# truemeat001/Simple-Raytracing-Render

Measured on AMD Instinct MI355X. Metric: Msamples/s (rays x bounces) + HBM GB/s vs roofline, Cornell+teapot 1024spp, higher is better.
Workload: dtype f32

## Files before the change

simple-raytracing-render_amd/csrc/kernels.h:

```cpp
#pragma once
#include <hip/hip_runtime.h>

#include <cstdint>

#include "device_scene.h"

namespace srr {

struct SceneView {
  const DObj* objs;
  int n_world;
  int has_media;
  const DXform* xforms;
  const DSphere* spheres;
  const DRect* rects;
  const DStandaloneTri* stris;
  const DMesh* meshes;
  const float4* nodes;
  const float4* node4;
  int node4_lds;
  int node4_total;
  const float4* node4q;
  int node4_lds_q;
  int use_q;
// ... 72 lines not shown
  UDiv31 div_spp, div_nx;
  uint64_t base_seed;
  int64_t n_paths;
  int max_depth;
  unsigned long long* cursor;
  unsigned long long* counters;
  float* sample;
  float* raw;
  uint8_t* rays;
  int keep_spp, keep_s0;
  float4* rec;
  int lanes;
  int* err;
  int stack_cap;
  int2* gstack;
  int gstack_cap;
  unsigned long long* wave_times;
  int deep_tries;
  float* slow_rays;
  unsigned* slow_count;
  int walk_q;
};
#ifndef SRR_KSTACK
#define SRR_KSTACK 8
#endif
constexpr int kPathsLdsStack = SRR_KSTACK;
constexpr int kPathsGlobalStack = 56;

constexpr int kPathsWorldLdsBytes = 8192;
#ifndef SRR_LDS_NODES
#define SRR_LDS_NODES 96
#endif
constexpr int kPathsLdsNodes = SRR_LDS_NODES;
void dump_trace_timing();
int paths_lanes_per_device(const SceneView& S, int device);
int paths_block_lanes(const SceneView& S);
int launch_paths(const SceneView& S, const PathWork& W, int all_families, hipStream_t st);
struct KatTables {
  const DCamera* cams;
  const DRect* rects;
  const DSphere* spheres;
  const DStandaloneTri* stris;
  const DLight* lights;
  int n_lights;
  const DObj* objs;
  const DXform* xforms;
  const DMedium* media;
  const DMat* mats;
  const DTex* texs;
  const uint8_t* images;
  const float* perlin_ranvec;
  const int32_t* perlin_perm;
  const int32_t* base;
};
int launch_kat(int kind, int n, int w, float* d_rec, const float* d_aux, const DStandaloneTri* d_tris,
               const KatTables& kt);
enum LibmId : int {
  kLibmRsin, kLibmRcos, kLibmRexp, kLibmRlog, kLibmRpow, kLibmRacos, kLibmRasin, kLibmRatan2, kLibmRdiv,
  kLibmSincosf, kLibmAtanf, kLibmSin64, kLibmCos64, kLibmSincos64, kLibmAcos64, kLibmAtan2_64, kLibmLog64,
  kLibmOcmlLog, kLibmOcmlSin, kLibmOcmlCos, kLibmOcmlPow5
};
struct LibmFn {
  LibmId id;
  const char* name;
  int f64, n_in, n_out;
};
// ... 61 lines not shown
```

simple-raytracing-render_amd/csrc/kernels.hip:

```cpp
#include <hip/hip_runtime.h>

#include <cfloat>
#include <algorithm>
#include <cstdint>
#include <cstdlib>
#include <cstring>

#include "device_scene.h"
#include "devmath.h"
#include "kernels.h"
#include "../../include/srr/merl.h"

namespace srr {
namespace dev {

SRR_D V3 sphere_center(const DSphere& s, float tm, bool moving) {
  V3 c0 = v3(s.c0[0], s.c0[1], s.c0[2]);
  if (!moving) return c0;
  V3 c1 = v3(s.c1[0], s.c1[1], s.c1[2]);
  return c0 + ((tm - s.t0) / (s.t1 - s.t0)) * (c1 - c0);
}

SRR_D bool sphere_hit(const DSphere& s, bool moving, const Ray& r, float tmin, float tmax, float& t) {
  V3 oc = r.o - sphere_center(s, r.tm, moving);
// ... 2524 lines not shown
      emitted = hit_emitted(S, mat, rdir, v3(hp.x, hp.y, hp.z), v3(hn.x, hn.y, hn.z), hp.w, hn.w);
    }
    finish_path(P, p, emitted, depth, spec, max_depth);
    return false;
  }
  float4 hp = ntl(&P.hit_p[p]), hn = ntl(&P.hit_n[p]);
  V3 hpt = v3(hp.x, hp.y, hp.z), nrm = v3(hn.x, hn.y, hn.z);
  const DMat M = S.mats[mat];
  Rng rng{ntl(&P.lcg[p]), ntl(&P.pcg[p])};
  V3 ndir;
  float ntime;
  float4 rec;
  bool sp;
  scatter<F>(S, M, rdir, ro.w, hpt, nrm, hp.w, hn.w, rng, rec, sp, ndir, ntime);
  nts(&P.rec_a[(size_t)p * max_depth + depth], rec);
  if (sp) spec |= (1ull << depth);
  nts(&P.ray_o[p], make_float4(hpt.x, hpt.y, hpt.z, ntime));
  nts(&P.ray_d[p], make_float4(ndir.x, ndir.y, ndir.z, 0.f));
  nts(&P.lcg[p], rng.lcg);
  nts(&P.pcg[p], rng.pcg);
  nts(&P.depth[p], depth + 1);
  nts(&P.spec[p], spec);
  return true;
}

SRR_D float4 rec_load(const float4* p) { return *p; }

constexpr int kPathsBlock = 256;
constexpr unsigned long long kPoolChunk = 64;

#ifndef SRR_DIAG_VARIANTS
#define SRR_DIAG_VARIANTS 0
#endif
constexpr int kRingWords = 11;

constexpr int kPathsLdsNodesBig =
    (160 * 1024 - 8192 - 8 * kPathsLdsStack * 1024 - 1024 - 4 * kRingWords * 1024) / 128;
constexpr int kPathsLdsNodesSmall = 8;

SRR_D void path_camera_ray(const SceneView& S, const PathWork& W, uint32_t idx, Ray& r, Rng& rng) {
  const uint32_t lp = udiv31(idx, W.div_spp), s = idx - lp * (uint32_t)W.spp_w;
  if ((int)lp >= W.npix || (int)s >= W.spp_w) atomicOr(W.err, 1);
  const int pix = W.pixels ? W.pixels[lp] : lp;
  V3 o, d;
  float tm;
  double sx, sy;
  sobol2_point((uint32_t)(W.s_base + (int)s), sx, sy);
  camera_ray(S, pix, W.s_base + s, sx, sy, W.nx, W.ny, W.base_seed, o, d, tm, rng, &W.div_nx);
  r = Ray{o, d, tm};
}

template <int BS>
SRR_D void ring_put(lds_ptr<float> e, const Ray& r, const Rng& rng) {
  e[0] = r.o.x;
  e[BS] = r.o.y;
  e[2 * BS] = r.o.z;
  e[3 * BS] = r.d.x;
  e[4 * BS] = r.d.y;
  e[5 * BS] = r.d.z;
  e[6 * BS] = r.tm;
  e[7 * BS] = __uint_as_float((uint32_t)rng.lcg);
  e[8 * BS] = __uint_as_float((uint32_t)(rng.lcg >> 32));
  e[9 * BS] = __uint_as_float((uint32_t)rng.pcg);
  e[10 * BS] = __uint_as_float((uint32_t)(rng.pcg >> 32));
}

template <int BS>
SRR_D void ring_get(lds_ptr<const float> e, Ray& r, Rng& rng) {
  r = Ray{v3(e[0], e[BS], e[2 * BS]), v3(e[3 * BS], e[4 * BS], e[5 * BS]), e[6 * BS]};
  rng.lcg = (uint64_t)__float_as_uint(e[7 * BS]) | ((uint64_t)__float_as_uint(e[8 * BS]) << 32);
  rng.pcg = (uint64_t)__float_as_uint(e[9 * BS]) | ((uint64_t)__float_as_uint(e[10 * BS]) << 32);
}

struct PathsArgs {
  SceneView S;
  PathWork W;
};
#if defined(__HIP_DEVICE_COMPILE__)
template <class T>
using kptr = const __attribute__((address_space(4))) T*;
SRR_D kptr<PathsArgs> paths_args() {
  kptr<PathsArgs> p = (kptr<PathsArgs>)__builtin_amdgcn_kernarg_segment_ptr();
  asm volatile("" : "+s"(p));
  return p;
}
#else
SRR_D const PathsArgs* paths_args() { return nullptr; }
#endif

template <bool MEDIA, bool ALLFAM, int MINB, bool TIMED = false, bool WL = true, bool QUAD = false, bool CQ = false,
          int BS = kPathsBlock, bool SP = false>
#ifdef SRR_NUM_VGPR
#define SRR_PATHS_VGPR_ATTR __attribute__((amdgpu_num_vgpr(SRR_NUM_VGPR)))
#else
#define SRR_PATHS_VGPR_ATTR
#endif
__global__ void __launch_bounds__(BS, MINB) SRR_PATHS_VGPR_ATTR k_paths(PathsArgs A) {
  static_assert(BS == kPathsBlock || BS == 1024, "block size");
  (void)A;
  uint64_t tp[8] = {0, 0, 0, 0, 0, 0, 0, 0};
  uint64_t tf[20] = {0, 0, 0, 0, 0, 0, 0, 0, 0, 0, 0, 0, 0, 0, 0, 0, 0, 0, 0, 0};
  uint64_t it = 0;
  constexpr int TR = TR_BVH4_PRUNE | (WL ? TR_WL : 0) | (QUAD ? TR_QUAD : 0) | (CQ ? TR_Q : 0) | (BS == 1024 ? TR_BIG : 0) |
                     ((SP && !QUAD && !CQ) ? TR_SUSP : 0);
  __shared__ uint4 s_world[WL ? kWorldLdsBytes / 16 : 1];
  const auto view = [&]() {
    SceneView S = paths_args()->S;
    if constexpr (WL) {
      const char* b = (const char*)s_world;
      S.objs = (const DObj*)(b + S.world_off[0]);
      S.xforms = (const DXform*)(b + S.world_off[1]);
      S.spheres = (const DSphere*)(b + S.world_off[2]);
      S.rects = (const DRect*)(b + S.world_off[3]);
      S.stris = (const DStandaloneTri*)(b + S.world_off[4]);
      S.meshes = (const DMesh*)(b + S.world_off[5]);
      S.media = (const DMedium*)(b + S.world_off[6]);
      S.mats = (const DMat*)(b + S.world_off[7]);
      S.texs = (const DTex*)(b + S.world_off[8]);
      S.lights = (const DLight*)(b + S.world_off[9]);
    }
    return S;
  };
  const auto work = []() { return PathWork(paths_args()->W); };
  __shared__ int s_node[kStack * BS];
  __shared__ float s_t[kStack * BS];
  constexpr bool RING = !QUAD;
  constexpr int kNodesLds = BS == 1024 ? kPathsLdsNodesBig : ((WL && RING) ? kPathsLdsNodesSmall : kPathsLdsNodes);
  __shared__ float4 s_n4[kNodesLds * 8];
  __shared__ float s_ring[RING ? kRingWords * BS : 1];
  const lds_ptr<float> ringw = to_lds(s_ring + (RING ? (threadIdx.x & ~63u) : 0));
  uint32_t ring_base = 0;
  const uint32_t n_paths = (uint32_t)paths_args()->W.n_paths;
  const uint64_t t_start = paths_args()->W.wave_times ? __builtin_amdgcn_s_memrealtime() : 0;
  {
    const SceneView S0 = paths_args()->S;
    if constexpr (WL)
      for (int i = threadIdx.x; i < S0.world_words; i += blockDim.x) s_world[i] = S0.world_blob[i];
    const int n_lds_nodes = CQ ? min(S0.node4_total, 2 * kNodesLds) : min(S0.node4_total, kNodesLds);
    if (CQ)
      for (int i = threadIdx.x; i < n_lds_nodes * 4; i += blockDim.x) s_n4[i] = S0.node4q[i];
    else
      for (int i = threadIdx.x; i < n_lds_nodes * 8; i += blockDim.x) s_n4[i] = S0.node4[i];
  }
  __syncthreads();
  const int slot = blockIdx.x * blockDim.x + threadIdx.x;
  const auto rec_at = [&](const PathWork& W, int k) -> float4* {
    int s = slot;
    asm volatile("" : "+v"(s));
    return W.rec + ((size_t)k * W.lanes + s);
  };
  int g = -1;
  uint32_t pool = 0, pool_end = 0;
  uint32_t nxt_lane0 = 0;
  bool nxt_armed = false;
  uint32_t nxt_base = 0;
  bool nxt_ready = false;
  Ray r{};
  Rng rng{};
  int depth = 0;
  int walking = 0;
  uint32_t nrays = 0;
  uint32_t n_events = 0;
  constexpr uint32_t kCapped = 1, kSuspended = 1u << 12;
  uint32_t n_iter = 0, max_rounds = 0;
  for (;;) {
    ++n_iter;
    uint64_t tq = TIMED ? __builtin_amdgcn_s_memtime() : 0;
    const bool need = g < 0;
    const uint64_t nm = __ballot(need);
    if (nm && pool < n_paths) {
      const SceneView S = view();
      const PathWork W = work();
      const uint32_t cnt = __popcll(nm);
      const uint32_t rank = __popcll(nm & ((1ull << lane_id()) - 1));
      const uint32_t avail = pool_end - pool;
      uint32_t idx = 0;
      if (RING) {
        if (need && rank < avail) {
          const uint32_t i0 = pool + rank;
          if (i0 < n_paths) {
            g = (int)i0;
            ring_get<BS>(ringw + (i0 - ring_base), r, rng);
            depth = 0;
          }
        }
        if (avail >= cnt) {
          pool += cnt;
        } else {
          uint32_t nb;
          if (nxt_armed) {
            nb = nxt_ready ? nxt_base : __builtin_amdgcn_readfirstlane(nxt_lane0);
            nxt_armed = false;
            nxt_ready = false;
          } else {
            uint32_t b = 0;
            if (lane_id() == 0) b = (uint32_t)atomicAdd(W.cursor, (unsigned long long)kPoolChunk);
            nb = __builtin_amdgcn_readfirstlane(b);
          }
          const uint32_t gi = nb + (uint32_t)lane_id();
          if (gi < n_paths) {
// ... 22 lines not shown
        uint32_t nb;
        if (nxt_armed) {
          nb = nxt_ready ? nxt_base : __builtin_amdgcn_readfirstlane(nxt_lane0);
          nxt_armed = false;
          nxt_ready = false;
        } else {
          uint32_t b = 0;
          if (lane_id() == 0) b = (uint32_t)atomicAdd(W.cursor, (unsigned long long)kPoolChunk);
          nb = __builtin_amdgcn_readfirstlane(b);
        }
        idx = rank < avail ? pool + rank : nb + (rank - avail);
        pool = nb + (cnt - avail);
        pool_end = nb + (uint32_t)kPoolChunk;
      }
      if (!RING && need && idx < n_paths) {
        g = (int)idx;
        path_camera_ray(S, W, idx, r, rng);
        depth = 0;
      }
    }
    if (!nxt_armed && pool_end < n_paths) {
      if (lane_id() == 0) nxt_lane0 = (uint32_t)atomicAdd(paths_args()->W.cursor, (unsigned long long)kPoolChunk);
      nxt_armed = true;
    }
    if (__ballot(g >= 0) == 0) break;
    if (TIMED) tf[9] += __popcll(__ballot(g >= 0));
    if (TIMED) {
      __builtin_amdgcn_s_waitcnt(0);
      const uint64_t t = __builtin_amdgcn_s_memtime();
      tp[0] += t - tq;
      tq = t;
      ++it;
    }
    bool done = false;
    V3 C = v3(0.f);
    bool diff = false, pend = false;
    int natt = 0;
    uint64_t fam_dt[3] = {0, 0, 0};
    DiffSetup ds{};
    V3 d_atten = v3(0.f), d_n = v3(0.f), d_dir = v3(0.f);
    float d_pdf = 0;
    int d_tries = 0;
    bool d_dead = false;
    WorldHit w{-1, -1, 0};
    if (g >= 0) {
      const SceneView S = view();
      const PathWork W = work();
      TraceCtx cx{nullptr, to_lds(s_node + threadIdx.x), to_lds(s_t + threadIdx.x)};
      cx.lds_nodes = (const __attribute__((address_space(3))) f32x4*)to_lds(s_n4);
      cx.lds_count = CQ ? min(S.node4_total, 2 * kNodesLds) : min(S.node4_total, kNodesLds);
      cx.st_cap = min(W.stack_cap, kStack);
      cx.ovf = W.counters + 11;
      cx.gst = W.gstack;
      cx.gst_cap = W.gstack ? W.gstack_cap : 0;
      cx.gst_stride = W.lanes;
      cx.slot = slot;
      if constexpr ((TR & TR_SUSP) != 0) {
        cx.walk_thr = vreg((int)((__popcll(__ballot(true)) * (uint32_t)paths_args()->W.walk_q) >> 6));
        cx.resume = walking;
        cx.susp = vreg(0);
      }
#ifdef SRR_SLOW_RAYS
      const uint64_t t_w0 = __builtin_amdgcn_s_memrealtime();
      cx.last_steps = 0;
      const Ray r_in = r;
#endif
      w = world_hit<MEDIA, TIMED ? (TR_BVH4_TIMED | (WL ? TR_WL : 0) | (SP ? TR_SUSP : 0)) : TR>(S, r, rng, cx);
      if constexpr ((TR & TR_SUSP) != 0) {
        walking = cx.susp;
        if (walking) {
          w.obj = -1;
          n_events += kSuspended;
        }
      }
#ifdef SRR_SLOW_RAYS
      const uint64_t t_w = __builtin_amdgcn_s_memrealtime() - t_w0;
      if ((t_w > (uint64_t)SRR_SLOW_RAYS || (cx.last_steps & (1 << 28))) && W.slow_rays) {
        const unsigned q = atomicAdd(W.slow_count, 1u);
        if (q < 65536u) {
          float* e = W.slow_rays + 16 * (size_t)q;
          e[0] = __int_as_float(g);
          e[1] = __int_as_float(depth);
          e[2] = r_in.o.x; e[3] = r_in.o.y; e[4] = r_in.o.z;
          e[5] = r_in.d.x; e[6] = r_in.d.y; e[7] = r_in.d.z;
          e[8] = r_in.tm;
          e[9] = __int_as_float((int)t_w);
          e[10] = __int_as_float(cx.last_steps);
          e[11] = __int_as_float(w.obj);
          e[12] = __int_as_float(w.prim);
          e[13] = w.t;
          e[14] = __int_as_float(slot);
          e[15] = __int_as_float((int)(t_w0 & 0x7fffffff));
        }
      }
#endif
      if (TIMED) {
        const uint64_t t = __builtin_amdgcn_s_memtime();
        tp[1] += t - tq - cx.mesh_cycles;
        tp[2] += cx.mesh_cycles;
        tf[10] += cx.mesh_steps;
        tf[11] += cx.mesh_lane_steps;
        tf[12] += cx.mesh_walkers;
        tf[13] += cx.leaf_cycles;
        tf[14] += cx.leaf_passes;
        tf[15] += cx.step_parts[0];
        tf[16] += cx.step_parts[1];
        tf[17] += cx.step_parts[2];
        tq = t;
      }
      done = !walking;
    }
    if (nxt_armed && !nxt_ready) {
      nxt_base = __builtin_amdgcn_readfirstlane(nxt_lane0);
      nxt_ready = true;
    }
    if (g >= 0) {
      if (w.obj >= 0) {
        const SceneView S = view();
        const PathWork W = work();
        const HitRec h = world_record<TR>(S, r, w);
        const int kind = h.mat >= 0 ? S.mats[h.mat].kind : -1;
        if (TIMED) {
          __builtin_amdgcn_s_waitcnt(0);
          const uint64_t t = __builtin_amdgcn_s_memtime();
          tp[5] += t - tq;
          tq = t;
        }
        const int fam = family_of(h.mat, kind, depth, W.max_depth);
        if (TIMED) {
          const uint64_t mb = __ballot(fam == FAM_BECK), ms = __ballot(fam == FAM_SPEC),
                         md = __ballot(fam == FAM_DIFF && S.n_lights > 0);
          tf[3] += mb != 0; tf[4] += ms != 0; tf[5] += md != 0;
          tf[6] += __popcll(mb); tf[7] += __popcll(ms); tf[8] += __popcll(md);
        }
        if (fam == FAM_TERM) {
          C = hit_emitted(S, h.mat, r.d, h.p, h.n, h.u, h.v);
        } else if ((!ALLFAM || fam == FAM_DIFF) && S.n_lights > 0) {
          const DMat M = S.mats[h.mat];
          d_atten = tex_value(S, M.tex, h.u, h.v, h.p);
          Bsdf f;
          f.kind = M.kind;
          f.n = h.n;
          f.uvw = onb_from_w(h.n);
          f.A = M.p[0];
          f.B = M.p[1];
          bsdf_prepare<false>(f, r.d);
          ds = diff_setup(f, h.p);
          d_dead = bsdf_dead(S, f, h.p);
          (void)drand(rng);
// ... 31 lines not shown
        sum += __shfl_xor(sum, o);
        mx = max(mx, __shfl_xor(mx, o));
      }
      tf[18] += sum;
      tf[19] += mx;
      for (int q = 0; q < 3; ++q) {
        uint64_t m = fam_dt[q];
        for (int o = 32; o > 0; o >>= 1) m = max(m, (uint64_t)__shfl_xor((unsigned long long)m, o));
        tf[q] += m;
      }
    }
    if (__ballot(pend)) {
      const SceneView S = view();
      const uint64_t tc = TIMED ? __builtin_amdgcn_s_memtime() : 0;
      int rounds = skip_mixture(S, ds, d_dead, pend, d_tries, rng.lcg, d_dir, d_pdf, 1);
      if (__ballot(pend)) rounds += coop_mixture(S, ds, pend, d_tries, rng.lcg, d_dir, d_pdf, paths_args()->W.deep_tries);
      if (TIMED) {
        tp[6] += __builtin_amdgcn_s_memtime() - tc;
        tp[7] += rounds;
      }
      max_rounds = max(max_rounds, (uint32_t)rounds);
    }
    if (diff) {
      const PathWork W = work();
      if (d_pdf == 0) n_events += kCapped;
      float c = dot(d_n, unit_vector(d_dir));
      if (c < 0) c = 0;
      const V3 as = d_atten * (c / kPi);
      if (depth >= W.max_depth || slot >= W.lanes) atomicOr(W.err, 2);
      else *rec_at(W, depth) = make_float4(as.x, as.y, as.z, d_pdf);
      r = Ray{ds.p, d_dir, r.tm};
      ++depth;
    }
    if (g >= 0) {
      const PathWork W = work();
      if (TIMED) {
        const uint64_t t = __builtin_amdgcn_s_memtime();
        tp[3] += t - tq;
        tq = t;
      }
      if (done && (g >= W.n_paths || depth > W.max_depth)) {
        atomicOr(W.err, 4);
        g = -1;
        done = false;
      }
      if (done) {
        int k = depth - 1;
        for (; k >= 0; k -= 4) {
          float4 a[4];
#pragma unroll
          for (int j = 0; j < 4; ++j) a[j] = k - j >= 0 ? rec_load(rec_at(W, k - j)) : make_float4(0, 0, 0, 0);
#pragma unroll
          for (int j = 0; j < 4; ++j) {
            if (k - j < 0) break;
            const V3 av = v3(a[j].x, a[j].y, a[j].z);
            if (__float_as_uint(a[j].w) == kSpecMark) C = av * C;
            else C = v3(0.f) + (av * C) / a[j].w;
          }
        }
        if (W.raw) {
          const size_t kq = (size_t)(g / W.spp_w) * W.keep_spp + W.keep_s0 + (size_t)(g % W.spp_w);
          W.raw[3 * kq] = C.x;
          W.raw[3 * kq + 1] = C.y;
          W.raw[3 * kq + 2] = C.z;
          W.rays[kq] = (uint8_t)(depth + 1);
        }
        if (!(C.x == C.x)) C.x = 0;
        if (!(C.y == C.y)) C.y = 0;
        if (!(C.z == C.z)) C.z = 0;
        nts(&W.sample[3 * (size_t)g], C.x);
        nts(&W.sample[3 * (size_t)g + 1], C.y);
        nts(&W.sample[3 * (size_t)g + 2], C.z);
        nrays += depth + 1;
        g = -1;
      }
      if (TIMED) tp[4] += __builtin_amdgcn_s_memtime() - tq;
    }
  }
  const PathWork W = work();
  if (TIMED && lane_id() == 0) {
    for (int q = 0; q < 5; ++q) atomicAdd(W.counters + 4 + q, (unsigned long long)tp[q]);
    atomicAdd(W.counters + 9, (unsigned long long)it);
    atomicAdd(W.counters + 10, (unsigned long long)tp[5]);
    atomicAdd(W.counters + 13, (unsigned long long)tp[6]);
    atomicAdd(W.counters + 14, (unsigned long long)tp[7]);
    for (int q = 0; q < 20; ++q) atomicAdd(W.counters + 16 + q, (unsigned long long)tf[q]);
  }

  unsigned long long tot = nrays;
  for (int o = 32; o > 0; o >>= 1) tot += __shfl_xor(tot, o);
  if (lane_id() == 0 && tot) atomicAdd(W.counters, tot);
  if (__ballot(n_events != 0)) {
    unsigned long long cap = n_events & (kSuspended - 1), su = n_events / kSuspended;
    for (int o = 32; o > 0; o >>= 1) {
      cap += __shfl_xor(cap, o);
      su += __shfl_xor(su, o);
    }
    if (lane_id() == 0) {
      if (cap) atomicAdd(W.counters + 15, cap);
      if (su) atomicAdd(W.counters + 36, su);
    }
  }
  if (W.wave_times && lane_id() == 0) {
    const size_t wv = (size_t)(blockIdx.x * blockDim.x + threadIdx.x) / 64;
    W.wave_times[4 * wv] = t_start;
    W.wave_times[4 * wv + 1] = __builtin_amdgcn_s_memrealtime();
    W.wave_times[4 * wv + 2] = tot;
    W.wave_times[4 * wv + 3] = n_iter | ((unsigned long long)max_rounds << 32);
  }
}

constexpr int kAccChunk = 16;
struct AccOut {
  float* out;
  int scale_ns;
};
SRR_D void acc_write(float* acc, AccOut o, size_t a, float cx, float cy, float cz) {
  acc[a] = cx;
  acc[a + 1] = cy;
// ... 823 lines not shown
  hipLaunchKernelGGL(dev::k_aov_eval, dim3((n + 255) / 256), dim3(256), 0, st, S, P, n, val);
}
void launch_aov_fold(const AovFold& A, hipStream_t st) {
  const int64_t g = (8 * (int64_t)A.np + 255) / 256;
  hipLaunchKernelGGL(dev::k_aov_fold, dim3((unsigned)g), dim3(256), 0, st, A.val, A.np, A.spp_b, A.acc, A.init,
                     A.finish, A.ns, A.p0, A.albedo, A.normal, A.depth);
}

void launch_scatter_pixels(const float* packed, const int32_t* index, int64_t n, float* image, hipStream_t st) {
  if (n <= 0) return;
  const int64_t g = (3 * n + 255) / 256;
  hipLaunchKernelGGL(dev::k_scatter_pixels, dim3((unsigned)g), dim3(256), 0, st, packed, index, n, image);
}


constexpr int kPathsOccDefault = 4;
static int paths_min_blocks() {
  static const int v = [] {
    const char* e = getenv("SRR_PATHS_OCC");
    int x = e ? atoi(e) : kPathsOccDefault;
    return x >= 2 && x <= 6 ? x : kPathsOccDefault;
  }();
  return v;
}

struct PathsVariant {
  bool media, allfam;
  bool wl;
  bool quad;
  bool sp;
  bool timing;
  bool cq;
  int bs;
};
static PathsVariant paths_variant(const SceneView& S, int all_families, int walk_q) {
  static const bool big = [] {
    const char* e = getenv("SRR_BIGBLOCK");
    return !e || atoi(e) != 0;
  }();
  static const bool timing = getenv("SRR_PATHS_TIMING") != nullptr;
  static const bool force_global = getenv("SRR_WORLD_GLOBAL") != nullptr;
  PathsVariant v;
  v.media = S.has_media != 0;
  v.allfam = all_families != 0;
  v.wl = !force_global && S.world_words * 16 <= dev::kWorldLdsBytes;
  v.quad = S.quad_trace != 0;
  v.sp = walk_q > 0;
  v.timing = timing;
  const bool timed = SRR_DIAG_VARIANTS && timing;
  v.cq = SRR_DIAG_VARIANTS && S.use_q && !S.quad_trace && !timed;
  v.bs = (big && v.wl && !timed && !S.quad_trace && S.node4_total > 0 && paths_min_blocks() == kPathsOccDefault)
             ? 1024
             : dev::kPathsBlock;
  return v;
}

int paths_block_lanes(const SceneView& S) { return paths_variant(S, 0, 0).bs; }

int paths_lanes_per_device(const SceneView& S, int device) {
  (void)S;
  int cus = 0, per_cu = 0;
  if (hipDeviceGetAttribute(&cus, hipDeviceAttributeMultiprocessorCount, device) != hipSuccess || cus <= 0) cus = 256;
  if (hipOccupancyMaxActiveBlocksPerMultiprocessor(&per_cu, (const void*)dev::k_paths<false, false, 4>,
                                                   dev::kPathsBlock, 0) != hipSuccess || per_cu <= 0)
    per_cu = 2;
  per_cu = std::max(per_cu, paths_min_blocks());
  return cus * per_cu * dev::kPathsBlock;
}

template <bool M, bool A, int MINB, bool TIMED = false, bool WL = true, bool QUAD = false, bool CQ = false,
          int BS = dev::kPathsBlock, bool SP = false>
static void launch_k_paths(const dev::PathsArgs& args, hipStream_t st) {
  hipLaunchKernelGGL((dev::k_paths<M, A, MINB, TIMED, WL, QUAD, CQ, BS, SP>), dim3(args.W.lanes / BS), dim3(BS), 0, st,
                     args);
}

template <bool M, bool A>
static void launch_paths_global(const PathsVariant& v, const dev::PathsArgs& args, hipStream_t st) {
  if (v.quad) return launch_k_paths<M, A, 4, false, false, true>(args, st);
  launch_k_paths<M, A, 4, false, false>(args, st);
}
// ... 1 lines not shown
template <bool M, bool A, int B>
static void launch_paths_lds(const PathsVariant& v, const dev::PathsArgs& args, hipStream_t st) {
#if SRR_DIAG_VARIANTS
  if (v.timing && v.sp) return launch_k_paths<M, A, 4, true, true, false, false, dev::kPathsBlock, true>(args, st);
  if (v.timing) return launch_k_paths<M, A, 4, true>(args, st);
#endif
  if constexpr (B == 4) {
#if SRR_DIAG_VARIANTS
    if (v.cq && v.bs == 1024) return launch_k_paths<M, A, 4, false, true, false, true, 1024>(args, st);
    if (v.cq) return launch_k_paths<M, A, 4, false, true, false, true>(args, st);
#endif
    if (v.bs == 1024 && !v.quad && v.sp) return launch_k_paths<M, A, 4, false, true, false, false, 1024, true>(args, st);
    if (v.bs == 1024 && !v.quad) return launch_k_paths<M, A, 4, false, true, false, false, 1024>(args, st);
    if (v.quad) return launch_k_paths<M, A, 4, false, true, true>(args, st);
  }
  launch_k_paths<M, A, B>(args, st);
}

template <bool M, bool A>
static void launch_paths_lds_occ(const PathsVariant& v, const dev::PathsArgs& args, hipStream_t st) {
#ifdef SRR_OCC_VARIANTS
  switch (paths_min_blocks()) {
    case 2: return launch_paths_lds<M, A, 2>(v, args, st);
    case 3: return launch_paths_lds<M, A, 3>(v, args, st);
    case 5: return launch_paths_lds<M, A, 5>(v, args, st);
    case 6: return launch_paths_lds<M, A, 6>(v, args, st);
  }
#endif
  launch_paths_lds<M, A, 4>(v, args, st);
}

int launch_paths(const SceneView& S, const PathWork& W, int all_families, hipStream_t st) {
  if (W.stack_cap < 1 || W.stack_cap > dev::kStack) return -1;
  const dev::PathsArgs args{S, W};
  const PathsVariant v = paths_variant(S, all_families, W.walk_q);
  if (!SRR_DIAG_VARIANTS && v.wl && (S.use_q || v.timing))
    fprintf(stderr, "srr: SRR_CBVH / SRR_PATHS_TIMING need the diagnostics build (make diag); ignored\n");
  if (!v.wl) {
    if (v.media && v.allfam) launch_paths_global<true, true>(v, args, st);
    else if (v.media) launch_paths_global<true, false>(v, args, st);
    else if (v.allfam) launch_paths_global<false, true>(v, args, st);
    else launch_paths_global<false, false>(v, args, st);
  } else {
    if (v.media && v.allfam) launch_paths_lds_occ<true, true>(v, args, st);
    else if (v.media) launch_paths_lds_occ<true, false>(v, args, st);
    else if (v.allfam) launch_paths_lds_occ<false, true>(v, args, st);
    else launch_paths_lds_occ<false, false>(v, args, st);
  }
  return 0;
}

int launch_merl_lookup(const double* table, int64_t n, const double* angles, double* rgb, int32_t* cell) {
  if (n <= 0) return 0;
  hipLaunchKernelGGL(dev::k_merl_lookup, dim3((unsigned)((n + 255) / 256)), dim3(256), 0, 0, table, n, angles, rgb,
                     cell);
  return hipGetLastError() == hipSuccess ? 0 : -5;
}

int launch_kat(int kind, int n, int w, float* d_rec, const float* d_aux, const DStandaloneTri* d_tris,
               const KatTables& kt) {
  const int blocks = kind >= dev::KAT_SPHERE ? n : (n + 63) / 64;
  hipLaunchKernelGGL(dev::k_kat, dim3(blocks), dim3(64), 0, 0, kind, n, w, d_rec, d_aux, d_tris, kt);
  return hipGetLastError() == hipSuccess ? 0 : -5;
}

int launch_libm(int fn, int64_t n, const void* d_x, const void* d_y, void* d_out0, void* d_out1) {
  if (fn < 0 || fn >= kLibmFnCount || n <= 0 || n > (int64_t)1 << 30) return -1;
  const dim3 g((unsigned)((n + 255) / 256));
// ... 48 lines not shown
```

simple-raytracing-render_amd/csrc/renderer.cpp:

```cpp
#include "renderer.h"

#include "multi.h"

#include <algorithm>
#include <chrono>
#include <cstdlib>
#include <cstring>
#include <memory>
#include <thread>
#include <cstdio>

namespace srr {

constexpr int kCtrWords = 40;
constexpr int kVisitWords = 3 + 2 * 64;

#define RCHK(x)                                                        \
  do {                                                                 \
    hipError_t e_ = (x);                                               \
    if (e_ != hipSuccess) {                                            \
      err = std::string(#x) + ": " + hipGetErrorString(e_);            \
      return SRR_EIO;                                                  \
    }                                                                  \
  } while (0)

template <class T>
static hipError_t upload(T** dst, const std::vector<T>& v, std::vector<void*>& keep) {
  size_t bytes = std::max<size_t>(v.size() * sizeof(T), 16);
  hipError_t e = hipMalloc((void**)dst, bytes);
  if (e != hipSuccess) return e;
  keep.push_back(*dst);
  if (!v.empty()) e = hipMemcpy(*dst, v.data(), v.size() * sizeof(T), hipMemcpyHostToDevice);
  return e;
}

int renderer_create(const Scene& sc, int device, srr_renderer** out, std::string& err) {
  Flat F;
  int rc = flatten(sc, F, err);
  if (rc < 0) return rc;
  return renderer_create_flat(F, device, out, err);
}

int renderer_create_flat(const Flat& F, int device, srr_renderer** out, std::string& err) {
  std::unique_ptr<srr_renderer> r(new srr_renderer());
  r->device = device;
  if (const char* e = getenv("SRR_LANES")) r->n_lanes = std::max(1, std::min(kMaxLanes, atoi(e)));
  RCHK(hipSetDevice(device));
// ... 515 lines not shown

static int paths_finish(srr_renderer* r, FrameSlot& F, const srr_params* p, srr_stats* stats, std::string& err) {
  RCHK(hipStreamSynchronize(F.st));
  RCHK(hipGetLastError());
  srr_stats s{};
  double kernel_ms = 0;
  for (int wi = 0; wi < F.n_windows; ++wi) {
    float ms = 0;
    RCHK(hipEventElapsedTime(&ms, F.win_ev[2 * wi], F.win_ev[2 * wi + 1]));
    kernel_ms += ms;
  }
  unsigned long long ctr[kCtrWords];
  std::memcpy(ctr, F.ctr_host, sizeof(ctr));
  if (getenv("SRR_PATHS_TIMING") && ctr[9]) {
    const double it = (double)ctr[9];
    fprintf(stderr, "k_paths per wave-iteration (ticks): refill %.0f  world %.0f  mesh %.0f  record %.0f  scatter %.0f  fold %.0f  (%llu wave-iterations)\n",
            ctr[4] / it, ctr[5] / it, ctr[6] / it, ctr[10] / it, (ctr[7] - ctr[10]) / it, ctr[8] / it, ctr[9]);
    fprintf(stderr, "  scatter: mixture loop %.0f ticks, %.2f rounds per wave-iteration\n", ctr[13] / it, ctr[14] / it);
    auto per = [](unsigned long long a, unsigned long long b) { return b ? (double)a / (double)b : 0.0; };
    fprintf(stderr, "  families: beck %.0f ticks/it (runs in %.1f %% of its, %.1f lanes/run), spec %.0f (%.1f %%, %.1f), "
                    "diff set-up %.0f (%.1f %%, %.1f); lanes in a path %.1f of 64\n",
            ctr[16] / it, 100 * ctr[19] / it, per(ctr[22], ctr[19]), ctr[17] / it, 100 * ctr[20] / it,
            per(ctr[23], ctr[20]), ctr[18] / it, 100 * ctr[21] / it, per(ctr[24], ctr[21]), ctr[25] / it);
    fprintf(stderr, "  mesh: longest walk %.1f node steps/it, %.1f lane steps/it over %.1f walking lanes, "
                    "%.0f ticks per step of the longest walk\n",
            ctr[26] / it, ctr[27] / it, ctr[28] / it, per(ctr[6], ctr[26]));
    fprintf(stderr, "  mesh leaf queue: %.0f ticks/it, %.1f passes/it (%.0f ticks per pass)\n", ctr[29] / it,
            ctr[30] / it, per(ctr[29], ctr[30]));
    fprintf(stderr, "  mesh step parts (ticks/it): node fetch %.0f  slab + queue %.0f  order + push + pop %.0f\n",
            ctr[31] / it, ctr[32] / it, ctr[33] / it);
    fprintf(stderr, "  beckmann mixture: %.2f attempts per Beckmann scatter, %.2f for the wave's slowest lane per run\n",
            per(ctr[34], ctr[22]), per(ctr[35], ctr[19]));
    fprintf(stderr, "  suspended walks: %.2f lanes per wave-iteration\n", ctr[36] / it);
  }
#ifdef SRR_SLOW_RAYS
  if (r->pw_slow) {
    unsigned n = 0;
    RCHK(hipMemcpy(&n, r->pw_slow + 16 * 65536, sizeof(unsigned), hipMemcpyDeviceToHost));
    n = std::min(n, 65536u);
    std::vector<float> v(16 * (size_t)n);
    if (n) RCHK(hipMemcpy(v.data(), r->pw_slow, v.size() * sizeof(float), hipMemcpyDeviceToHost));
    auto I = [&](size_t k) { int x; memcpy(&x, &v[k], 4); return x; };
    for (unsigned i = 0; i < n; ++i) {
      const size_t b = 16 * (size_t)i;
      fprintf(stderr, "SLOWRAY {\"g\": %d, \"depth\": %d, \"o\": [%.9g, %.9g, %.9g], \"d\": [%.9g, %.9g, %.9g], "
              "\"tm\": %.9g, \"ticks\": %d, \"steps\": %d, \"obj\": %d, \"prim\": %d, \"t\": %.9g, \"slot\": %d, "
              "\"t0\": %d, \"spp_w\": %d}\n", I(b), I(b + 1), v[b + 2], v[b + 3], v[b + 4], v[b + 5], v[b + 6], v[b + 7], v[b + 8],
              I(b + 9), I(b + 10), I(b + 11), I(b + 12), v[b + 13], I(b + 14), I(b + 15), p->spp);
    }
  }
#else
  (void)r;
  (void)p;
#endif
  if (ctr[2]) {
    err = "k_paths index guard tripped (bits " + std::to_string(ctr[2]) + ")";
    return SRR_EIO;
  }
  float total = 0;
  RCHK(hipEventElapsedTime(&total, F.ev_beg, F.ev_end));
  s.world_rays = (int64_t)ctr[0];
  s.stack_overflows = (int64_t)ctr[11];
  s.deep_traversals = (int64_t)ctr[12];
  s.mixture_capped = (int64_t)ctr[15];
  s.walks_suspended = (int64_t)ctr[36];
  s.paths = F.paths;
// ... 706 lines not shown
```

Baseline: 9072.

## Pre-trace camera rays into the LDS ring with stored hits before shading

Adds a pre-trace mode for 1024-lane blocks (and timed builds) without media or all-families. When a wave refills its LDS ring with a new chunk of camera rays, it traces all of them together in a coherent pass and stores obj/prim/t in three extra ring words. Lanes that later pick up those paths start at shading with the hit already known. This batches the coherent primary rays instead of mixing them with divergent secondary bounces, and lets the loop run up to two shade rounds per iteration. The extra ring words cut the number of BVH nodes held in LDS for big blocks (344 to 248). The loop control also gets more complex, and new timing counters and an env knob to cap LDS nodes are added.

```diff
diff --git a/simple-raytracing-render_amd/csrc/kernels.h b/simple-raytracing-render_amd/csrc/kernels.h
--- a/simple-raytracing-render_amd/csrc/kernels.h
+++ b/simple-raytracing-render_amd/csrc/kernels.h
@@ -128,6 +128,44 @@
 #define SRR_LDS_NODES 96
 #endif
 constexpr int kPathsLdsNodes = SRR_LDS_NODES;
+
+constexpr int kRingRayWords = 11;
+constexpr int kRingHitWord = kRingRayWords;
+constexpr int kRingWordsHit = kRingHitWord + 3;
+constexpr int ring_words(bool pretrace) { return pretrace ? kRingWordsHit : kRingRayWords; }
+static_assert(ring_words(false) == 11 && ring_words(true) == 14 && kRingHitWord + 2 < kRingWordsHit, "ring entry layout");
+
+constexpr int kLdsPerCu = 160 * 1024;
+constexpr int paths_lds_fixed(int bs, bool wl) {
+  return (wl ? kPathsWorldLdsBytes : 16) + 8 * kPathsLdsStack * bs + bs;
+}
+constexpr int paths_lds_nodes_big(bool pretrace) {
+  return (kLdsPerCu - paths_lds_fixed(1024, true) - 4 * ring_words(pretrace) * 1024) / 128;
+}
+constexpr int paths_lds_nodes_global(bool pretrace) {
+  const int room = (kLdsPerCu / 4 - paths_lds_fixed(256, false) - 4 * ring_words(pretrace) * 256) / 128;
+  return room < kPathsLdsNodes ? room : kPathsLdsNodes;
+}
+constexpr int kPathsLdsNodesSmall = 8;
+constexpr int paths_lds_nodes(int bs, bool wl, bool ring, bool pretrace) {
+  return bs == 1024 ? paths_lds_nodes_big(pretrace)
+                    : (wl && ring) ? kPathsLdsNodesSmall : ring ? paths_lds_nodes_global(pretrace) : kPathsLdsNodes;
+}
+constexpr int paths_lds_bytes(int bs, bool wl, bool ring, bool pretrace) {
+  return (wl ? kPathsWorldLdsBytes : 16) + 8 * kPathsLdsStack * bs + 128 * paths_lds_nodes(bs, wl, ring, pretrace) +
+         (ring ? 4 * ring_words(pretrace) * bs : 4);
+}
+constexpr bool paths_lds_fits(int bs, bool wl, bool ring, bool pretrace) {
+  return paths_lds_nodes(bs, wl, ring, pretrace) >= 1 && paths_lds_bytes(bs, wl, ring, pretrace) <= (bs == 1024 ? kLdsPerCu : kLdsPerCu / 4);
+}
+#if SRR_KSTACK == 8 && SRR_LDS_NODES == 96
+static_assert(paths_lds_nodes_big(false) == 344 && paths_lds_nodes_big(true) == 248, "1,024-lane node sets");
+#endif
+static_assert(paths_lds_fits(1024, true, true, false) && paths_lds_fits(1024, true, true, true), "1,024-lane blocks: 160 KB");
+static_assert(paths_lds_fits(256, true, true, false) && paths_lds_fits(256, true, true, true) &&
+              paths_lds_fits(256, true, false, false), "256-lane blocks, world in LDS: 40 KB");
+static_assert(paths_lds_fits(256, false, true, false) && paths_lds_fits(256, false, true, true) &&
+              paths_lds_fits(256, false, false, false), "256-lane blocks, world in global memory: 40 KB");
 void dump_trace_timing();
 int paths_lanes_per_device(const SceneView& S, int device);
 int paths_block_lanes(const SceneView& S);
diff --git a/simple-raytracing-render_amd/csrc/kernels.hip b/simple-raytracing-render_amd/csrc/kernels.hip
--- a/simple-raytracing-render_amd/csrc/kernels.hip
+++ b/simple-raytracing-render_amd/csrc/kernels.hip
@@ -2580,12 +2580,6 @@
 #ifndef SRR_DIAG_VARIANTS
 #define SRR_DIAG_VARIANTS 0
 #endif
-constexpr int kRingWords = 11;
-
-constexpr int kPathsLdsNodesBig =
-    (160 * 1024 - 8192 - 8 * kPathsLdsStack * 1024 - 1024 - 4 * kRingWords * 1024) / 128;
-constexpr int kPathsLdsNodesSmall = 8;
-
 SRR_D void path_camera_ray(const SceneView& S, const PathWork& W, uint32_t idx, Ray& r, Rng& rng) {
   const uint32_t lp = udiv31(idx, W.div_spp), s = idx - lp * (uint32_t)W.spp_w;
   if ((int)lp >= W.npix || (int)s >= W.spp_w) atomicOr(W.err, 1);
@@ -2620,6 +2614,17 @@
   rng.pcg = (uint64_t)__float_as_uint(e[9 * BS]) | ((uint64_t)__float_as_uint(e[10 * BS]) << 32);
 }
 
+template <int BS>
+SRR_D void ring_put_hit(lds_ptr<float> e, int obj, int prim, float t) {
+  e[kRingHitWord * BS] = __int_as_float(obj);
+  e[(kRingHitWord + 1) * BS] = __int_as_float(prim);
+  e[(kRingHitWord + 2) * BS] = t;
+}
+template <int BS>
+SRR_D void ring_get_ray(lds_ptr<const float> e, Ray& r) {
+  r = Ray{v3(e[0], e[BS], e[2 * BS]), v3(e[3 * BS], e[4 * BS], e[5 * BS]), e[6 * BS]};
+}
+
 struct PathsArgs {
   SceneView S;
   PathWork W;
@@ -2648,6 +2653,7 @@
   (void)A;
   uint64_t tp[8] = {0, 0, 0, 0, 0, 0, 0, 0};
   uint64_t tf[20] = {0, 0, 0, 0, 0, 0, 0, 0, 0, 0, 0, 0, 0, 0, 0, 0, 0, 0, 0, 0};
+  uint64_t tz[2] = {0, 0};
   uint64_t it = 0;
   constexpr int TR = TR_BVH4_PRUNE | (WL ? TR_WL : 0) | (QUAD ? TR_QUAD : 0) | (CQ ? TR_Q : 0) | (BS == 1024 ? TR_BIG : 0) |
                      ((SP && !QUAD && !CQ) ? TR_SUSP : 0);
@@ -2673,9 +2679,15 @@
   __shared__ int s_node[kStack * BS];
   __shared__ float s_t[kStack * BS];
   constexpr bool RING = !QUAD;
-  constexpr int kNodesLds = BS == 1024 ? kPathsLdsNodesBig : ((WL && RING) ? kPathsLdsNodesSmall : kPathsLdsNodes);
+  constexpr bool PT = RING && !MEDIA && !ALLFAM && (BS == 1024 || TIMED);
+  constexpr int kRingWords = ring_words(PT);
+  constexpr int kNodesLds = paths_lds_nodes(BS, WL, RING, PT);
+  static_assert(paths_lds_fits(BS, WL, RING, PT), "k_paths LDS");
   __shared__ float4 s_n4[kNodesLds * 8];
   __shared__ float s_ring[RING ? kRingWords * BS : 1];
+  static_assert(sizeof(s_world) + sizeof(s_node) + sizeof(s_t) + sizeof(s_n4) + sizeof(s_ring) ==
+                    (size_t)paths_lds_bytes(BS, WL, RING, PT), "k_paths LDS as kernels.h counts it");
+  const auto lds_nodes = [](const SceneView& S) { return min(S.node4_total, (CQ ? 2 : 1) * kNodesLds); };
   const lds_ptr<float> ringw = to_lds(s_ring + (RING ? (threadIdx.x & ~63u) : 0));
   uint32_t ring_base = 0;
   const uint32_t n_paths = (uint32_t)paths_args()->W.n_paths;
@@ -2684,7 +2696,7 @@
     const SceneView S0 = paths_args()->S;
     if constexpr (WL)
       for (int i = threadIdx.x; i < S0.world_words; i += blockDim.x) s_world[i] = S0.world_blob[i];
-    const int n_lds_nodes = CQ ? min(S0.node4_total, 2 * kNodesLds) : min(S0.node4_total, kNodesLds);
+    const int n_lds_nodes = lds_nodes(S0);
     if (CQ)
       for (int i = threadIdx.x; i < n_lds_nodes * 4; i += blockDim.x) s_n4[i] = S0.node4q[i];
     else
@@ -2711,9 +2723,15 @@
   uint32_t n_events = 0;
   constexpr uint32_t kCapped = 1, kSuspended = 1u << 12;
   uint32_t n_iter = 0, max_rounds = 0;
+  constexpr int kNoHit = -2;
+  WorldHit w{kNoHit, -1, 0};
+  bool fill = false;
+  uint64_t tpt[3] = {0, 0, 0};
   for (;;) {
     ++n_iter;
     uint64_t tq = TIMED ? __builtin_amdgcn_s_memtime() : 0;
+    if constexpr (!PT) {
+    w = WorldHit{-1, -1, 0};
     const bool need = g < 0;
     const uint64_t nm = __ballot(need);
     if (nm && pool < n_paths) {
@@ -2802,23 +2820,26 @@
       tq = t;
       ++it;
     }
-    bool done = false;
-    V3 C = v3(0.f);
-    bool diff = false, pend = false;
-    int natt = 0;
-    uint64_t fam_dt[3] = {0, 0, 0};
-    DiffSetup ds{};
-    V3 d_atten = v3(0.f), d_n = v3(0.f), d_dir = v3(0.f);
-    float d_pdf = 0;
-    int d_tries = 0;
-    bool d_dead = false;
-    WorldHit w{-1, -1, 0};
-    if (g >= 0) {
+    }
+    const bool fill_now = PT && fill;
+    bool act = g >= 0 && (!PT || w.obj == kNoHit);
+    Ray tr = r;
+    if constexpr (PT) {
+      if (fill_now) {
+        act = ring_base + (uint32_t)lane_id() < n_paths && !walking;
+        if (act) ring_get_ray<BS>(ringw + lane_id(), tr);
+      }
+      if (TIMED) {
+        tf[9] += __popcll(__ballot(g >= 0));
+        ++it;
+      }
+    }
+    if (act) {
       const SceneView S = view();
       const PathWork W = work();
       TraceCtx cx{nullptr, to_lds(s_node + threadIdx.x), to_lds(s_t + threadIdx.x)};
       cx.lds_nodes = (const __attribute__((address_space(3))) f32x4*)to_lds(s_n4);
-      cx.lds_count = CQ ? min(S.node4_total, 2 * kNodesLds) : min(S.node4_total, kNodesLds);
+      cx.lds_count = lds_nodes(S);
       cx.st_cap = min(W.stack_cap, kStack);
       cx.ovf = W.counters + 11;
       cx.gst = W.gstack;
@@ -2826,21 +2847,27 @@
       cx.gst_stride = W.lanes;
       cx.slot = slot;
       if constexpr ((TR & TR_SUSP) != 0) {
-        cx.walk_thr = vreg((int)((__popcll(__ballot(true)) * (uint32_t)paths_args()->W.walk_q) >> 6));
-        cx.resume = walking;
+        cx.walk_thr = vreg(fill_now ? 0 : (int)((__popcll(__ballot(true)) * (uint32_t)paths_args()->W.walk_q) >> 6));
+        cx.resume = fill_now ? vreg(0) : walking;
         cx.susp = vreg(0);
       }
 #ifdef SRR_SLOW_RAYS
       const uint64_t t_w0 = __builtin_amdgcn_s_memrealtime();
       cx.last_steps = 0;
-      const Ray r_in = r;
+      const Ray r_in = tr;
 #endif
-      w = world_hit<MEDIA, TIMED ? (TR_BVH4_TIMED | (WL ? TR_WL : 0) | (SP ? TR_SUSP : 0)) : TR>(S, r, rng, cx);
-      if constexpr ((TR & TR_SUSP) != 0) {
-        walking = cx.susp;
-        if (walking) {
-          w.obj = -1;
-          n_events += kSuspended;
+      const WorldHit wh =
+          world_hit<MEDIA, TIMED ? (TR_BVH4_TIMED | (WL ? TR_WL : 0) | (SP ? TR_SUSP : 0)) : TR>(S, tr, rng, cx);
+      if (fill_now) {
+        ring_put_hit<BS>(ringw + lane_id(), wh.obj, wh.prim, wh.t);
+      } else {
+        w = wh;
+        if constexpr ((TR & TR_SUSP) != 0) {
+          walking = cx.susp;
+          if (walking) {
+            w.obj = PT ? kNoHit : -1;
+            n_events += kSuspended;
+          }
         }
       }
 #ifdef SRR_SLOW_RAYS
@@ -2856,9 +2883,9 @@
           e[8] = r_in.tm;
           e[9] = __int_as_float((int)t_w);
           e[10] = __int_as_float(cx.last_steps);
-          e[11] = __int_as_float(w.obj);
-          e[12] = __int_as_float(w.prim);
-          e[13] = w.t;
+          e[11] = __int_as_float(wh.obj);
+          e[12] = __int_as_float(wh.prim);
+          e[13] = wh.t;
           e[14] = __int_as_float(slot);
           e[15] = __int_as_float((int)(t_w0 & 0x7fffffff));
         }
@@ -2866,25 +2893,114 @@
 #endif
       if (TIMED) {
         const uint64_t t = __builtin_amdgcn_s_memtime();
-        tp[1] += t - tq - cx.mesh_cycles;
-        tp[2] += cx.mesh_cycles;
-        tf[10] += cx.mesh_steps;
-        tf[11] += cx.mesh_lane_steps;
-        tf[12] += cx.mesh_walkers;
-        tf[13] += cx.leaf_cycles;
-        tf[14] += cx.leaf_passes;
-        tf[15] += cx.step_parts[0];
-        tf[16] += cx.step_parts[1];
-        tf[17] += cx.step_parts[2];
+        if (fill_now) {
+          tpt[0] += t - tq;
+          ++tpt[1];
+        } else {
+          if (__ballot(depth != 0) == 0) {
+            tz[0] += t - tq;
+            ++tz[1];
+          }
+          tp[1] += t - tq - cx.mesh_cycles;
+          tp[2] += cx.mesh_cycles;
+          tf[10] += cx.mesh_steps;
+          tf[11] += cx.mesh_lane_steps;
+          tf[12] += cx.mesh_walkers;
+          tf[13] += cx.leaf_cycles;
+          tf[14] += cx.leaf_passes;
+          tf[15] += cx.step_parts[0];
+          tf[16] += cx.step_parts[1];
+          tf[17] += cx.step_parts[2];
+        }
         tq = t;
       }
-      done = !walking;
+    }
+    if constexpr (PT) {
+      if (fill_now) {
+        __builtin_amdgcn_fence(__ATOMIC_SEQ_CST, "wavefront");
+        fill = false;
+      }
     }
     if (nxt_armed && !nxt_ready) {
       nxt_base = __builtin_amdgcn_readfirstlane(nxt_lane0);
       nxt_ready = true;
     }
-    if (g >= 0) {
+#pragma nounroll
+    for (int round = 0; round < (PT ? 2 : 1); ++round) {
+    if constexpr (PT) {
+      if (TIMED) tq = __builtin_amdgcn_s_memtime();
+      const bool need = g < 0;
+      const uint64_t nm = __ballot(need);
+      if (nm && pool < n_paths) {
+        const uint32_t cnt = __popcll(nm);
+        const uint32_t rank = __popcll(nm & ((1ull << lane_id()) - 1));
+        const uint32_t avail = pool_end - pool;
+        if (need && rank < avail) {
+          const uint32_t i0 = pool + rank;
+          if (i0 < n_paths) {
+            const lds_ptr<const float> e = ringw + (i0 - ring_base);
+            g = (int)i0;
+            ring_get<BS>(e, r, rng);
+            w = WorldHit{__float_as_int(e[kRingHitWord * BS]), __float_as_int(e[(kRingHitWord + 1) * BS]),
+                         e[(kRingHitWord + 2) * BS]};
+            depth = 0;
+          }
+        }
+        if (avail >= cnt) {
+          pool += cnt;
+        } else {
+          const SceneView S = view();
+          const PathWork W = work();
+          uint32_t nb;
+          if (nxt_armed) {
+            nb = nxt_ready ? nxt_base : __builtin_amdgcn_readfirstlane(nxt_lane0);
+            nxt_armed = false;
+            nxt_ready = false;
+          } else {
+            uint32_t b = 0;
+            if (lane_id() == 0) b = (uint32_t)atomicAdd(W.cursor, (unsigned long long)kPoolChunk);
+            nb = __builtin_amdgcn_readfirstlane(b);
+          }
+          __builtin_amdgcn_fence(__ATOMIC_SEQ_CST, "wavefront");
+          const uint32_t gi = nb + (uint32_t)lane_id();
+          if (gi < n_paths) {
+            Ray gr;
+            Rng grng;
+            path_camera_ray(S, W, gi, gr, grng);
+            ring_put<BS>(ringw + lane_id(), gr, grng);
+            ring_put_hit<BS>(ringw + lane_id(), kNoHit, -1, 0.f);
+          }
+          __builtin_amdgcn_fence(__ATOMIC_SEQ_CST, "wavefront");
+          ring_base = nb;
+          pool = nb;
+          pool_end = nb + (uint32_t)kPoolChunk;
+          fill = nb < n_paths;
+        }
+      }
+      if (TIMED) {
+        __builtin_amdgcn_s_waitcnt(0);
+        const uint64_t t = __builtin_amdgcn_s_memtime();
+        tp[0] += t - tq;
+        tq = t;
+      }
+      if (fill) break;
+    }
+    const bool sh = g >= 0 && (!PT || w.obj != kNoHit);
+    if constexpr (PT) {
+      if (__ballot(sh) == 0) break;
+      if (TIMED) ++tpt[2];
+    }
+    bool done = sh && (PT || !walking);
+    V3 C = v3(0.f);
+    bool diff = false, pend = false;
+    int natt = 0;
+    uint64_t fam_dt[3] = {0, 0, 0};
+    DiffSetup ds{};
+    V3 d_atten = v3(0.f), d_n = v3(0.f), d_dir = v3(0.f);
+    float d_pdf = 0;
+    int d_tries = 0;
+    bool d_dead = false;
+    if (sh) {
       if (w.obj >= 0) {
         const SceneView S = view();
         const PathWork W = work();
@@ -2982,8 +3098,9 @@
       r = Ray{ds.p, d_dir, r.tm};
       ++depth;
     }
-    if (g >= 0) {
+    if (sh) {
       const PathWork W = work();
+      if (PT) w.obj = kNoHit;
       if (TIMED) {
         const uint64_t t = __builtin_amdgcn_s_memtime();
         tp[3] += t - tq;
@@ -3026,6 +3143,14 @@
       }
       if (TIMED) tp[4] += __builtin_amdgcn_s_memtime() - tq;
     }
+    }
+    if constexpr (PT) {
+      if (!nxt_armed && pool_end < n_paths) {
+        if (lane_id() == 0) nxt_lane0 = (uint32_t)atomicAdd(paths_args()->W.cursor, (unsigned long long)kPoolChunk);
+        nxt_armed = true;
+      }
+      if (!fill && pool >= n_paths && __ballot(g >= 0) == 0) break;
+    }
   }
   const PathWork W = work();
   if (TIMED && lane_id() == 0) {
@@ -3035,6 +3160,8 @@
     atomicAdd(W.counters + 13, (unsigned long long)tp[6]);
     atomicAdd(W.counters + 14, (unsigned long long)tp[7]);
     for (int q = 0; q < 20; ++q) atomicAdd(W.counters + 16 + q, (unsigned long long)tf[q]);
+    for (int q = 0; q < 2; ++q) atomicAdd(W.counters + 37 + q, (unsigned long long)tz[q]);
+    for (int q = 0; q < 3; ++q) atomicAdd(W.counters + 39 + q, (unsigned long long)tpt[q]);
   }
 
   unsigned long long tot = nrays;
@@ -3924,6 +4051,7 @@
   bool timing;
   bool cq;
   int bs;
+  int lds_nodes_cap;
 };
 static PathsVariant paths_variant(const SceneView& S, int all_families, int walk_q) {
   static const bool big = [] {
@@ -3932,6 +4060,8 @@
   }();
   static const bool timing = getenv("SRR_PATHS_TIMING") != nullptr;
   static const bool force_global = getenv("SRR_WORLD_GLOBAL") != nullptr;
+  const char* nc_env = getenv("SRR_LDS_NODES_CAP");
+  const int nodes_cap = nc_env ? std::max(0, atoi(nc_env)) : 0;
   PathsVariant v;
   v.media = S.has_media != 0;
   v.allfam = all_families != 0;
@@ -3939,6 +4069,7 @@
   v.quad = S.quad_trace != 0;
   v.sp = walk_q > 0;
   v.timing = timing;
+  v.lds_nodes_cap = nodes_cap;
   const bool timed = SRR_DIAG_VARIANTS && timing;
   v.cq = SRR_DIAG_VARIANTS && S.use_q && !S.quad_trace && !timed;
   v.bs = (big && v.wl && !timed && !S.quad_trace && S.node4_total > 0 && paths_min_blocks() == kPathsOccDefault)
@@ -4006,8 +4137,9 @@
 
 int launch_paths(const SceneView& S, const PathWork& W, int all_families, hipStream_t st) {
   if (W.stack_cap < 1 || W.stack_cap > dev::kStack) return -1;
-  const dev::PathsArgs args{S, W};
+  dev::PathsArgs args{S, W};
   const PathsVariant v = paths_variant(S, all_families, W.walk_q);
+  if (v.lds_nodes_cap > 0) args.S.node4_total = std::min(args.S.node4_total, v.lds_nodes_cap);
   if (!SRR_DIAG_VARIANTS && v.wl && (S.use_q || v.timing))
     fprintf(stderr, "srr: SRR_CBVH / SRR_PATHS_TIMING need the diagnostics build (make diag); ignored\n");
   if (!v.wl) {
diff --git a/simple-raytracing-render_amd/csrc/renderer.cpp b/simple-raytracing-render_amd/csrc/renderer.cpp
--- a/simple-raytracing-render_amd/csrc/renderer.cpp
+++ b/simple-raytracing-render_amd/csrc/renderer.cpp
@@ -12,7 +12,7 @@
 
 namespace srr {
 
-constexpr int kCtrWords = 40;
+constexpr int kCtrWords = 48;
 constexpr int kVisitWords = 3 + 2 * 64;
 
 #define RCHK(x)                                                        \
@@ -594,6 +594,12 @@
     fprintf(stderr, "  beckmann mixture: %.2f attempts per Beckmann scatter, %.2f for the wave's slowest lane per run\n",
             per(ctr[34], ctr[22]), per(ctr[35], ctr[19]));
     fprintf(stderr, "  suspended walks: %.2f lanes per wave-iteration\n", ctr[36] / it);
+    fprintf(stderr, "  camera-ray-only iterations (every tracing lane at depth 0): %llu of %llu, world + mesh %.0f ticks "
+                    "per wave-iteration of them; the others %.0f\n",
+            ctr[38], ctr[9], per(ctr[37], ctr[38]), per(ctr[5] + ctr[6] - ctr[37], ctr[9] - ctr[38]));
+    fprintf(stderr, "  pre-trace: %llu passes of the %llu wave-iterations, %.0f ticks each (%.0f per wave-iteration); "
+                    "shade rounds %.2f per wave-iteration\n",
+            ctr[40], ctr[9], per(ctr[39], ctr[40]), ctr[39] / it, ctr[41] / it);
   }
 #ifdef SRR_SLOW_RAYS
   if (r->pw_slow) {
```

New measurement: 9329 (median of 6 runs). +2.8%, better.
